# kelaendi/mused

Hardware: AMD Instinct MI355X
Metric: stream rows/sec, d=1024 l=128 window=10k synthetic (SWFD + kNN similarity + eigenstep + labels) (higher is better)
Workload: dtype f64; 1 GPU; synthetic d=1024 l=128 window=10000 k=50 (BASELINE config 2); stream=blob, W=10000, d=1024, l=128, k=50, modalities=1, swfd_levels=14, rccl_ranks=1, lanes_per_gpu=20, padded_window_slots=2

## Files before the change

mused_amd/csrc/gemm_f64.h:

```cpp
#pragma once
#include <mutex>
#include "common.h"

namespace mused {

typedef double v4f64 __attribute__((ext_vector_type(4)));

constexpr int GEMM_BM = 128;
constexpr int GEMM_BN = 128;
constexpr int GEMM_BK = 16;
constexpr int GEMM_LD = 144;
constexpr int GEMM_THREADS = 256;
constexpr int GEMM_LDS_BYTES = 2  * 2  * GEMM_BK * GEMM_LD * 8;

struct GemmArgs {
  const void* A;
  const void* B;
  long lda, ldb;
  long strideA, strideB;
  int M, N, K;
  int kchunk;
  int splitk;
  int bsplit;
  int tiles_m, tiles_n;
  const int* rep;
  const int* list;
  const int* kact;
  int sym;
};

template <typename TIn, bool VEC>
__device__ __forceinline__ void stage_load_kc(const TIn* __restrict__ src, long ld, int r0, int nrows, int k0,
                                              int kend, TIn (&r)[8]) {
  const int m = threadIdx.x & 127;
  const int kh = threadIdx.x >> 7;
  const int row = r0 + m;
  const int k = k0 + kh * 8;
  if (row < nrows) {
    const TIn* p = src + (long)row * ld + k;
    if (VEC && k + 8 <= kend) {
      if (sizeof(TIn) == 4) {
        const float4 a = *reinterpret_cast<const float4*>(p);
        const float4 b = *reinterpret_cast<const float4*>(p + 4);
        r[0] = a.x; r[1] = a.y; r[2] = a.z; r[3] = a.w;
        r[4] = b.x; r[5] = b.y; r[6] = b.z; r[7] = b.w;
      } else {
        const double2* q = reinterpret_cast<const double2*>(p);
#pragma unroll
        for (int j = 0; j < 4; ++j) {
          const double2 v = q[j];
          r[2 * j] = v.x;
          r[2 * j + 1] = v.y;
        }
      }
    } else {
#pragma unroll
      for (int j = 0; j < 8; ++j) r[j] = (k + j < kend) ? p[j] : (TIn)0;
    }
  } else {
#pragma unroll
    for (int j = 0; j < 8; ++j) r[j] = (TIn)0;
  }
}

template <typename TIn>
__device__ __forceinline__ void stage_store_kc(double* __restrict__ lds, const TIn (&r)[8]) {
  const int m = threadIdx.x & 127;
  const int kh = threadIdx.x >> 7;
#pragma unroll
  for (int j = 0; j < 8; ++j) lds[(kh * 8 + j) * GEMM_LD + m] = (double)r[j];
}

template <typename TIn, bool VEC>
__device__ __forceinline__ void stage_load_mc(const TIn* __restrict__ src, long ld, int c0, int ncols, int k0,
                                              int kend, TIn (&r)[8]) {
  const int kk = threadIdx.x >> 4;
  const int c = c0 + (threadIdx.x & 15) * 8;
  const int k = k0 + kk;
  if (k < kend) {
    const TIn* p = src + (long)k * ld + c;
    if (VEC && c + 8 <= ncols) {
      if (sizeof(TIn) == 4) {
        const float4 a = *reinterpret_cast<const float4*>(p);
        const float4 b = *reinterpret_cast<const float4*>(p + 4);
        r[0] = a.x; r[1] = a.y; r[2] = a.z; r[3] = a.w;
        r[4] = b.x; r[5] = b.y; r[6] = b.z; r[7] = b.w;
      } else {
        const double2* q = reinterpret_cast<const double2*>(p);
#pragma unroll
        for (int j = 0; j < 4; ++j) {
          const double2 v = q[j];
          r[2 * j] = v.x;
          r[2 * j + 1] = v.y;
        }
      }
    } else {
#pragma unroll
      for (int j = 0; j < 8; ++j) r[j] = (c + j < ncols) ? p[j] : (TIn)0;
    }
  } else {
#pragma unroll
    for (int j = 0; j < 8; ++j) r[j] = (TIn)0;
  }
}

template <typename TIn>
__device__ __forceinline__ void stage_store_mc(double* __restrict__ lds, const TIn (&r)[8]) {
  const int kk = threadIdx.x >> 4;
  const int c = (threadIdx.x & 15) * 8;
  double* p = lds + kk * GEMM_LD + c;
#pragma unroll
  for (int j = 0; j < 8; ++j) p[j] = (double)r[j];
}

template <typename TIn>
__device__ __forceinline__ void stage_load8(const TIn* __restrict__ p, TIn (&r)[8]) {
  if (sizeof(TIn) == 4) {
    const float4 a = *reinterpret_cast<const float4*>(p);
    const float4 b = *reinterpret_cast<const float4*>(p + 4);
    r[0] = a.x; r[1] = a.y; r[2] = a.z; r[3] = a.w;
    r[4] = b.x; r[5] = b.y; r[6] = b.z; r[7] = b.w;
  } else {
    const double2* q = reinterpret_cast<const double2*>(p);
#pragma unroll
    for (int j = 0; j < 4; ++j) {
      const double2 v = q[j];
      r[2 * j] = v.x;
      r[2 * j + 1] = v.y;
    }
  }
}
template <typename TIn>
__device__ __forceinline__ void stage_load_kc_full(const TIn* __restrict__ src, long ld, int r0, int k0, TIn (&r)[8]) {
  stage_load8(src + (long)(r0 + (threadIdx.x & 127)) * ld + k0 + (threadIdx.x >> 7) * 8, r);
}
template <typename TIn>
__device__ __forceinline__ void stage_load_mc_full(const TIn* __restrict__ src, long ld, int c0, int k0, TIn (&r)[8]) {
  stage_load8(src + (long)(k0 + (threadIdx.x >> 4)) * ld + c0 + (threadIdx.x & 15) * 8, r);
}

__device__ __forceinline__ int xcd_remap(int pid, int nwg) {
  const int q = nwg >> 3, r = nwg & 7, xcd = pid & 7;
  const int base = (xcd < r) ? xcd * (q + 1) : r * (q + 1) + (xcd - r) * q;
  return base + (pid >> 3);
}

template <typename TA, typename TB, bool A_KC, bool B_KC, bool VEC>
__device__ __forceinline__ void gemm_tile_mainloop(const GemmArgs& g, const TA* __restrict__ A, const TB* __restrict__ B,
                                                   int m0, int n0, int k_lo, int k_hi, double* smem,
                                                   v4f64 (&acc)[4][4]) {
  double* As = smem;
  double* Bs = smem + 2 * GEMM_BK * GEMM_LD;
  const int lane = threadIdx.x & 63;
  const int wave = threadIdx.x >> 6;
  const int wr = wave >> 1, wc = wave & 1;
  const int kq = lane >> 4, li = lane & 15;
#pragma unroll
  for (int i = 0; i < 4; ++i)
#pragma unroll
    for (int j = 0; j < 4; ++j) acc[i][j] = (v4f64){0.0, 0.0, 0.0, 0.0};

  TA ra[8];
  TB rb[8];
  const int nkt = (k_hi - k_lo + GEMM_BK - 1) / GEMM_BK;

  const bool full_mn = VEC && m0 + GEMM_BM <= g.M && n0 + GEMM_BN <= g.N;
  auto load_tile = [&](int kt) {
    const int k0 = k_lo + kt * GEMM_BK;
    if (full_mn && k0 + GEMM_BK <= k_hi) {
      if (A_KC) stage_load_kc_full<TA>(A, g.lda, m0, k0, ra); else stage_load_mc_full<TA>(A, g.lda, m0, k0, ra);
      if (B_KC) stage_load_kc_full<TB>(B, g.ldb, n0, k0, rb); else stage_load_mc_full<TB>(B, g.ldb, n0, k0, rb);
      return;
    }
    if (A_KC) stage_load_kc<TA, VEC>(A, g.lda, m0, g.M, k0, k_hi, ra);
    else      stage_load_mc<TA, VEC>(A, g.lda, m0, g.M, k0, k_hi, ra);
    if (B_KC) stage_load_kc<TB, VEC>(B, g.ldb, n0, g.N, k0, k_hi, rb);
    else      stage_load_mc<TB, VEC>(B, g.ldb, n0, g.N, k0, k_hi, rb);
  };
  auto store_tile = [&](int buf) {
    double* a = As + buf * GEMM_BK * GEMM_LD;
    double* b = Bs + buf * GEMM_BK * GEMM_LD;
    if (A_KC) stage_store_kc(a, ra); else stage_store_mc(a, ra);
    if (B_KC) stage_store_kc(b, rb); else stage_store_mc(b, rb);
  };

  if (nkt > 0) {
    load_tile(0);
    store_tile(0);
  }
  __syncthreads();

  int cur = 0;
  for (int kt = 0; kt < nkt; ++kt) {
    const bool more = (kt + 1 < nkt);
    if (more) load_tile(kt + 1);
    const double* a = As + cur * GEMM_BK * GEMM_LD + wr * 64 + li;
    const double* b = Bs + cur * GEMM_BK * GEMM_LD + wc * 64 + li;
#pragma unroll
    for (int kk = 0; kk < GEMM_BK / 4; ++kk) {
      double fa[4], fb[4];
#pragma unroll
      for (int i = 0; i < 4; ++i) fa[i] = a[(kk * 4 + kq) * GEMM_LD + i * 16];
#pragma unroll
      for (int j = 0; j < 4; ++j) fb[j] = b[(kk * 4 + kq) * GEMM_LD + j * 16];
#pragma unroll
      for (int i = 0; i < 4; ++i)
#pragma unroll
        for (int j = 0; j < 4; ++j)
          acc[i][j] = __builtin_amdgcn_mfma_f64_16x16x4f64(fa[i], fb[j], acc[i][j], 0, 0, 0);
    }
    if (more) store_tile(cur ^ 1);
    __syncthreads();
    cur ^= 1;
  }
}

template <typename TA, typename TB, bool A_KC, bool B_KC, bool VEC, typename Epi>
__global__ __launch_bounds__(GEMM_THREADS, 2) void gemm_f64_kernel(GemmArgs g, Epi epi) {
  extern __shared__ __attribute__((aligned(16))) double smem[];

  int z = blockIdx.z;
  int zb = g.bsplit ? z / g.bsplit : z;
  if (g.list) {
    if (zb >= g.list[0]) return;
    const int e = g.list[1 + zb];
    z += (e - zb) * (g.bsplit ? g.bsplit : 1);
    zb = e;
  } else if (g.rep && g.rep[zb] != zb) return;
  int tm, tn;
  if (g.sym) {
    const int t = g.tiles_n, nwg = t * (t + 1) / 2;
    const int e = xcd_remap(blockIdx.x, nwg);
    int r = (int)((2.0 * t + 1.0 - sqrt((2.0 * t + 1.0) * (2.0 * t + 1.0) - 8.0 * e)) * 0.5);
    r = r < 0 ? 0 : (r > t - 1 ? t - 1 : r);
    while (r > 0 && r * t - r * (r - 1) / 2 > e) --r;
    while (r + 1 < t && (r + 1) * t - (r + 1) * r / 2 <= e) ++r;
    tm = r;
    tn = r + (e - (r * t - r * (r - 1) / 2));
  } else {
    const int nwg = g.tiles_m * g.tiles_n;
    const int wg = xcd_remap(blockIdx.x, nwg);
    constexpr int GROUP_M = 8;
    const int per_group = GROUP_M * g.tiles_n;
    const int group_id = wg / per_group;
    const int first_m = group_id * GROUP_M;
    const int group_size = min(g.tiles_m - first_m, GROUP_M);
    tm = first_m + (wg % group_size);
    tn = (wg % per_group) / group_size;
  }
  const int m0 = tm * GEMM_BM, n0 = tn * GEMM_BN;
  const bool mirror = g.sym && tm != tn;

  int k_lo = 0, k_hi = g.K;
  const TA* A = reinterpret_cast<const TA*>(g.A);
  const TB* B = reinterpret_cast<const TB*>(g.B);
  if (g.splitk) {
    k_lo = z * g.kchunk;
    k_hi = min(g.K, k_lo + g.kchunk);
  } else {
    A += (long)zb * g.strideA;
    B += (long)zb * g.strideB;
    if (g.bsplit) {
      k_lo = (z - zb * g.bsplit) * g.kchunk;
      k_hi = min(g.K, k_lo + g.kchunk);
    } else if (g.kact) {
      k_hi = min(g.K, g.kact[zb]);
    }
  }

  const int lane = threadIdx.x & 63;
  const int wave = threadIdx.x >> 6;
  const int wr = wave >> 1, wc = wave & 1;
  const int kq = lane >> 4, li = lane & 15;

  v4f64 acc[4][4];
  gemm_tile_mainloop<TA, TB, A_KC, B_KC, VEC>(g, A, B, m0, n0, k_lo, k_hi, smem, acc);

#pragma unroll
  for (int i = 0; i < 4; ++i) {
#pragma unroll
    for (int j = 0; j < 4; ++j) {
      const int col = n0 + wc * 64 + j * 16 + li;
#pragma unroll
      for (int r = 0; r < 4; ++r) {
        const int row = m0 + wr * 64 + i * 16 + kq + 4 * r;
        if (row < g.M && col < g.N) epi(z, row, col, acc[i][j][r]);
      }
    }
  }
  if (mirror) {
    __syncthreads();
    double* patch = smem + wave * (32 * 65);
#pragma unroll
    for (int half = 0; half < 2; ++half) {
#pragma unroll
      for (int i = 0; i < 4; ++i)
#pragma unroll
        for (int jj = 0; jj < 2; ++jj) {
          const int j = half * 2 + jj;
          const int col = n0 + wc * 64 + j * 16 + li;
#pragma unroll
          for (int r = 0; r < 4; ++r) {
            const int rl = i * 16 + kq + 4 * r;
            const int rg = m0 + wr * 64 + rl;
            patch[(jj * 16 + li) * 65 + rl] = (rg < g.M && col < g.N) ? epi.value(col, rg, acc[i][j][r]) : 0.0;
          }
        }
      const int rowm = m0 + wr * 64 + lane;
#pragma unroll 8
      for (int c = 0; c < 32; ++c) {
        const int colm = n0 + wc * 64 + half * 32 + c;
        if (colm < g.N && rowm < g.M) epi.put(z, colm, rowm, patch[c * 65 + lane]);
      }
    }
  }
}

struct EpiStore {
  double* C;
  long ldc;
  long strideC;
  double alpha;
  __device__ __forceinline__ void operator()(int z, int row, int col, double v) const {
    C[(long)z * strideC + (long)row * ldc + col] = alpha * v;
  }
  __device__ __forceinline__ double value(int, int, double v) const { return alpha * v; }
  __device__ __forceinline__ void put(int z, int row, int col, double val) const {
    C[(long)z * strideC + (long)row * ldc + col] = val;
  }
};

template <typename TA, typename TB, bool A_KC, bool B_KC, bool VEC, typename Epi>
int gemm_f64_prepare_t() {
  static std::once_flag once;
  static hipError_t err = hipSuccess;
  std::call_once(once, [] {
    auto k = gemm_f64_kernel<TA, TB, A_KC, B_KC, VEC, Epi>;
    err = hipFuncSetAttribute(reinterpret_cast<const void*>(k), hipFuncAttributeMaxDynamicSharedMemorySize,
                              GEMM_LDS_BYTES);
  });
  MUSED_CHECK_HIP(err);
  return MUSED_OK;
}

template <typename TA, typename TB, bool A_KC, bool B_KC, typename Epi>
int gemm_f64_launch_t(GemmArgs g, int batch, Epi epi, bool vec, hipStream_t stream) {
  g.tiles_m = cdiv(g.M, GEMM_BM);
  g.tiles_n = cdiv(g.N, GEMM_BN);
  if (g.M <= 0 || g.N <= 0 || batch <= 0) return MUSED_OK;
  dim3 grid(g.sym ? g.tiles_n * (g.tiles_n + 1) / 2 : g.tiles_m * g.tiles_n, 1, batch);
  int rc;
  if (vec) {
    if ((rc = gemm_f64_prepare_t<TA, TB, A_KC, B_KC, true, Epi>())) return rc;
    hipLaunchKernelGGL((gemm_f64_kernel<TA, TB, A_KC, B_KC, true, Epi>), grid, dim3(GEMM_THREADS), GEMM_LDS_BYTES,
                       stream, g, epi);
  } else {
    if ((rc = gemm_f64_prepare_t<TA, TB, A_KC, B_KC, false, Epi>())) return rc;
    hipLaunchKernelGGL((gemm_f64_kernel<TA, TB, A_KC, B_KC, false, Epi>), grid, dim3(GEMM_THREADS), GEMM_LDS_BYTES,
                       stream, g, epi);
  }
  MUSED_LAUNCH_CHECK();
  return MUSED_OK;
}

template <typename T>
static inline bool vec_ok(const void* p, long ld, long stride) {
  const long e = 16 / (long)sizeof(T);
  return ((uintptr_t)p % 16 == 0) && (ld % e == 0) && (stride % e == 0);
}

}
```

Before: 625,700 rows/s.

## Compute only upper-triangle 16x16 blocks in diagonal tiles of symmetric GEMM

For symmetric (A·Aᵀ) GEMMs, diagonal 128x128 tiles now compute only the 36 upper-triangle 16x16 MFMA blocks. These are spread 9 per wave, and a single A tile is staged in LDS. Mirrored blocks are transposed through an LDS patch and written out via the epilogue's value/put interface. This removes the redundant lower-triangle MFMA work and B-tile staging on diagonal tiles. The cost is a more complex epilogue with extra LDS traffic, a per-wave switch, and a new requirement that Epi provide value() and put(). An environment variable can disable the path.

```diff
diff --git a/mused_amd/csrc/gemm_f64.h b/mused_amd/csrc/gemm_f64.h
--- a/mused_amd/csrc/gemm_f64.h
+++ b/mused_amd/csrc/gemm_f64.h
@@ -1,5 +1,7 @@
 #pragma once
+#include <cstdlib>
 #include <mutex>
+#include <type_traits>
 #include "common.h"
 
 namespace mused {
@@ -213,6 +215,153 @@
     __syncthreads();
     cur ^= 1;
   }
+}
+
+constexpr int DIAG_I[4][9] = {{0, 0, 1, 0, 1, 2, 0, 1, 2}, {3, 0, 1, 2, 3, 4, 0, 1, 2}, {3, 4, 5, 0, 1, 2, 3, 4, 5}, {6, 0, 1, 2, 3, 4, 5, 6, 7}};
+constexpr int DIAG_J[4][9] = {{0, 1, 1, 2, 2, 2, 3, 3, 3}, {3, 4, 4, 4, 4, 4, 5, 5, 5}, {5, 5, 5, 6, 6, 6, 6, 6, 6}, {6, 7, 7, 7, 7, 7, 7, 7, 7}};
+constexpr int DIAG_NF[4] = {4, 6, 7, 8};
+constexpr int DIAG_NGRP[4] = {3, 2, 2, 1};
+constexpr int DIAG_GRP[4][3][3] = {{{1, 0, 1}, {2, 0, 2}, {3, 0, 3}}, {{4, 0, 4}, {5, 0, 3}, {0, 0, 0}}, {{5, 3, 2}, {6, 0, 6}, {0, 0, 0}}, {{7, 0, 7}, {0, 0, 0}, {0, 0, 0}}};
+constexpr int DIAG_PATCH_LD = 130;
+
+constexpr int diag_acc_index(int w, int i, int j) {
+  for (int n = 0; n < 9; ++n)
+    if (DIAG_I[w][n] == i && DIAG_J[w][n] == j) return n;
+  return -1;
+}
+
+template <int W, int N = 0>
+__device__ __forceinline__ void diag_mfma9(const double (&f)[8], v4f64 (&acc)[9]) {
+  if constexpr (N < 9) {
+    constexpr int i = DIAG_I[W][N], j = DIAG_J[W][N];
+    acc[N] = __builtin_amdgcn_mfma_f64_16x16x4f64(f[i], f[j], acc[N], 0, 0, 0);
+    diag_mfma9<W, N + 1>(f, acc);
+  }
+}
+template <int W>
+__device__ __forceinline__ void diag_kstep(const double* __restrict__ a, v4f64 (&acc)[9]) {
+#pragma unroll
+  for (int kk = 0; kk < GEMM_BK / 4; ++kk) {
+    double f[8];
+#pragma unroll
+    for (int b = 0; b < 8; ++b) f[b] = (b < DIAG_NF[W]) ? a[kk * 4 * GEMM_LD + b * 16] : 0.0;
+    diag_mfma9<W>(f, acc);
+  }
+}
+
+template <typename TA, bool A_KC, bool VEC>
+__device__ __forceinline__ void gemm_tile_mainloop_diag(const GemmArgs& g, const TA* __restrict__ A, int m0, int k_lo, int k_hi,
+                                                        double* As, int wave, v4f64 (&acc)[9]) {
+  const int lane = threadIdx.x & 63;
+  const int kq = lane >> 4, li = lane & 15;
+#pragma unroll
+  for (int n = 0; n < 9; ++n) acc[n] = (v4f64){0.0, 0.0, 0.0, 0.0};
+
+  TA ra[8];
+  const int nkt = (k_hi - k_lo + GEMM_BK - 1) / GEMM_BK;
+  const bool full_m = VEC && m0 + GEMM_BM <= g.M;
+  auto load_tile = [&](int kt) {
+    const int k0 = k_lo + kt * GEMM_BK;
+    if (full_m && k0 + GEMM_BK <= k_hi) {
+      if (A_KC) stage_load_kc_full<TA>(A, g.lda, m0, k0, ra); else stage_load_mc_full<TA>(A, g.lda, m0, k0, ra);
+      return;
+    }
+    if (A_KC) stage_load_kc<TA, VEC>(A, g.lda, m0, g.M, k0, k_hi, ra);
+    else      stage_load_mc<TA, VEC>(A, g.lda, m0, g.M, k0, k_hi, ra);
+  };
+  auto store_tile = [&](int buf) {
+    double* a = As + buf * GEMM_BK * GEMM_LD;
+    if (A_KC) stage_store_kc(a, ra); else stage_store_mc(a, ra);
+  };
+
+  if (nkt > 0) {
+    load_tile(0);
+    store_tile(0);
+  }
+  __syncthreads();
+
+  int cur = 0;
+  for (int kt = 0; kt < nkt; ++kt) {
+    const bool more = (kt + 1 < nkt);
+    if (more) load_tile(kt + 1);
+    const double* a = As + cur * GEMM_BK * GEMM_LD + kq * GEMM_LD + li;
+    switch (wave) {
+      case 0: diag_kstep<0>(a, acc); break;
+      case 1: diag_kstep<1>(a, acc); break;
+      case 2: diag_kstep<2>(a, acc); break;
+      default: diag_kstep<3>(a, acc); break;
+    }
+    if (more) store_tile(cur ^ 1);
+    __syncthreads();
+    cur ^= 1;
+  }
+}
+
+template <int W, int GI, int II, typename Epi>
+__device__ __forceinline__ void diag_mirror_fill(const GemmArgs& g, const Epi& epi, int m0, double* patch, const v4f64 (&acc)[9]) {
+  constexpr int j = DIAG_GRP[W][GI][0], i0 = DIAG_GRP[W][GI][1], cnt = DIAG_GRP[W][GI][2];
+  if constexpr (II < cnt) {
+    constexpr int n = diag_acc_index(W, i0 + II, j);
+    static_assert(n >= 0, "block not held by this wave");
+    const int lane = threadIdx.x & 63;
+    const int kq = lane >> 4, li = lane & 15;
+    const int col = m0 + j * 16 + li;
+#pragma unroll
+    for (int r = 0; r < 4; ++r) {
+      const int rl = II * 16 + kq + 4 * r;
+      const int rg = m0 + i0 * 16 + rl;
+      patch[li * DIAG_PATCH_LD + rl] = (rg < g.M && col < g.N) ? epi.value(col, rg, acc[n][r]) : 0.0;
+    }
+    diag_mirror_fill<W, GI, II + 1>(g, epi, m0, patch, acc);
+  }
+}
+
+template <int W, int GI, typename Epi>
+__device__ __forceinline__ void diag_mirror_groups(const GemmArgs& g, const Epi& epi, int z, int m0, double* patch,
+                                                   const v4f64 (&acc)[9]) {
+  if constexpr (GI < DIAG_NGRP[W]) {
+    constexpr int j = DIAG_GRP[W][GI][0], i0 = DIAG_GRP[W][GI][1], cnt = DIAG_GRP[W][GI][2];
+    constexpr int width = cnt * 16;
+    const int lane = threadIdx.x & 63;
+    diag_mirror_fill<W, GI, 0>(g, epi, m0, patch, acc);
+#pragma unroll
+    for (int t = 0; t < width / 4; ++t) {
+      const int idx = t * 64 + lane;
+      const int c = idx / width, off = idx % width;
+      const int rowm = m0 + j * 16 + c, colm = m0 + i0 * 16 + off;
+      if (rowm < g.N && colm < g.M) epi.put(z, rowm, colm, patch[c * DIAG_PATCH_LD + off]);
+    }
+    diag_mirror_groups<W, GI + 1>(g, epi, z, m0, patch, acc);
+  }
+}
+
+template <int W, int N, typename Epi>
+__device__ __forceinline__ void diag_store_blocks(const GemmArgs& g, const Epi& epi, int z, int m0, const v4f64 (&acc)[9]) {
+  if constexpr (N < 9) {
+    const int lane = threadIdx.x & 63;
+    const int col = m0 + DIAG_J[W][N] * 16 + (lane & 15);
+#pragma unroll
+    for (int r = 0; r < 4; ++r) {
+      const int row = m0 + DIAG_I[W][N] * 16 + (lane >> 4) + 4 * r;
+      if (row < g.M && col < g.N) epi(z, row, col, acc[N][r]);
+    }
+    diag_store_blocks<W, N + 1>(g, epi, z, m0, acc);
+  }
+}
+
+template <int W, typename Epi>
+__device__ __forceinline__ void diag_epilogue(const GemmArgs& g, const Epi& epi, int z, int m0, double* smem,
+                                              const v4f64 (&acc)[9]) {
+  diag_store_blocks<W, 0>(g, epi, z, m0, acc);
+  diag_mirror_groups<W, 0>(g, epi, z, m0, smem + W * (16 * DIAG_PATCH_LD), acc);
+}
+
+inline int gemm_sym_diag_enabled() {
+  static const int on = [] {
+    const char* s = getenv("MUSED_GEMM_SYM_DIAG");
+    return (s && s[0] == '0') ? 0 : 1;
+  }();
+  return on;
 }
 
 template <typename TA, typename TB, bool A_KC, bool B_KC, bool VEC, typename Epi>
@@ -268,6 +417,21 @@
     }
   }
 
+  if constexpr (std::is_same<TA, TB>::value && A_KC == B_KC) {
+    if (g.sym == 2 && tm == tn) {
+      const int w = __builtin_amdgcn_readfirstlane(threadIdx.x >> 6);
+      v4f64 acc9[9];
+      gemm_tile_mainloop_diag<TA, A_KC, VEC>(g, A, m0, k_lo, k_hi, smem, w, acc9);
+      switch (w) {
+        case 0: diag_epilogue<0>(g, epi, z, m0, smem, acc9); break;
+        case 1: diag_epilogue<1>(g, epi, z, m0, smem, acc9); break;
+        case 2: diag_epilogue<2>(g, epi, z, m0, smem, acc9); break;
+        default: diag_epilogue<3>(g, epi, z, m0, smem, acc9); break;
+      }
+      return;
+    }
+  }
+
   const int lane = threadIdx.x & 63;
   const int wave = threadIdx.x >> 6;
   const int wr = wave >> 1, wc = wave & 1;
@@ -347,6 +511,7 @@
 int gemm_f64_launch_t(GemmArgs g, int batch, Epi epi, bool vec, hipStream_t stream) {
   g.tiles_m = cdiv(g.M, GEMM_BM);
   g.tiles_n = cdiv(g.N, GEMM_BN);
+  if (g.sym) g.sym = gemm_sym_diag_enabled() ? 2 : 1;
   if (g.M <= 0 || g.N <= 0 || batch <= 0) return MUSED_OK;
   dim3 grid(g.sym ? g.tiles_n * (g.tiles_n + 1) / 2 : g.tiles_m * g.tiles_n, 1, batch);
   int rc;
```

New measurement: 652,300 rows/s, median of 6. 1.04x the previous value.
